# jonaselgammal/GPry

Measured on AMD Instinct MI355X. Metric: gp_refit_plus_nora_acq_cycle_throughput, higher is better.
Workload: dtype f64

## Files before the change

gpry_amd/csrc/api.hip:

```cpp
#include "sweep.h"
#include "kb_gram.h"
#include <algorithm>

int require_model(gpry_ctx* ctx, bool need_factor) {
    if (ctx->N <= 0) return gpry_fail(ctx, -1, "no training set (call gpry_set_train)");
    if (!ctx->have_theta) return gpry_fail(ctx, -1, "no hyperparameters (call gpry_set_theta)");
    if (need_factor && !ctx->factor_valid) return gpry_fail(ctx, -1, "model not factorised (call gpry_factorize)");
    if (need_factor && ctx->tf.has_x_affine)
        for (int k = 0; k < ctx->d; k++)
            if (!(ctx->tf.x_span[k] != 0.0) || !isfinite(ctx->tf.x_span[k]) || !isfinite(ctx->tf.x_lo[k]))
                return gpry_fail(ctx, -1, "affine map of X: span %g, offset %g in dimension %d of %d (gpry_set_affine of another model?)",
                                 ctx->tf.x_span[k], ctx->tf.x_lo[k], k, ctx->d);
    return 0;
}


static int copy_out_matrix(gpry_ctx* ctx, const double* dsrc, int64_t ld, int64_t rows, int64_t cols, double* hdst) {
    HIP_TRY(ctx, hipMemcpy2DAsync(hdst, sizeof(double) * cols, dsrc, sizeof(double) * ld,
                                  sizeof(double) * cols, rows, hipMemcpyDeviceToHost, ctx->stream));
    HIP_TRY(ctx, hipStreamSynchronize(ctx->stream));
    return 0;
}

bool panel_timed_out(int marker) { return (marker & 0xFF00) == 0x5A00; }
// ... 42 lines not shown
                StageScope s(ctx, "trtri");
                if (piped) { GPRY_TRY(trtri_pipeline_finish(ctx)); guard.armed = false; }
                else GPRY_TRY(trtri_lower(ctx, A, V, T, ctx->Np));
            }
        }
    }
    ctx->info_cleared = false;
    if (!info_host) return 0;
    int info[4] = {0, 0, 0, 0};
    HIP_TRY(ctx, hipMemcpyAsync(info, ctx->dinfo, 4 * sizeof(int), hipMemcpyDeviceToHost, ctx->stream));
    HIP_TRY(ctx, hipStreamSynchronize(ctx->stream));
    if (panel_timed_out(info[3])) return panel_timeout_error(ctx, info[3]);
    *info_host = info[0] != 0 ? info[0] : info[1];
    return 0;
}

constexpr int RES_INFO = LML_RES_INFO;
static_assert(RES_INFO + 3 <= GPRY_BRES_STRIDE, "result row too short");
int lml_chain(gpry_ctx* ctx, int want_grad, double* dres) {
    GPRY_TRY(build_factor(ctx, ctx->dW, ctx->dW2, ctx->dW3, nullptr));
    double* dz = ctx->dvec;
    double* da = ctx->dvec + ctx->Np;
    double* dout = ctx->dvec + 2 * ctx->Np;
    {
        StageScope s(ctx, "solve_alpha");
        GPRY_TRY(solve_alpha(ctx, ctx->dW2, ctx->dy, dz, da, ctx->Np));
        GPRY_TRY(logdet_and_quad(ctx, ctx->dW, dz, ctx->Np, dout, want_grad ? nullptr : dres, RES_INFO));
    }
    if (!want_grad) return 0;
    {
        StageScope s(ctx, "lauum");
        GPRY_TRY(lauum_lower(ctx, ctx->dW2, ctx->dW3, ctx->Np));
    }
    StageScope s(ctx, "lml_traces");
    return launch_lml_traces(ctx, ctx->dW3, da, dout + 2, dout, dres, RES_INFO);
}

struct BatchLayout {
    int64_t w, w2, w3, xs, vec, part, split, par, info;
    int64_t part_cap, split_cap, stride;
};
static int batch_layout(gpry_ctx* ctx, const BatchChain& bc, BatchLayout* L) {
    const int64_t Np = ctx->Np, nn = Np * Np;
    int slices = 0;
    GPRY_TRY(factor_chain_slices(ctx, Np, &slices));
    const int DPsel = ctx->d <= 4 ? 4 : ctx->d <= 8 ? 8 : ctx->d <= 16 ? 16 : ctx->d <= 24 ? 24 : 32;
    const int64_t nb = Np / 64, ntile = nb * (nb + 1) / 2;
    const int64_t p1 = ((Np + 255) / 256) * Np, p2 = ntile * (DPsel + 2);
    int64_t o = 0;
    auto take = [&](int64_t n) { const int64_t at = o; o += round_up(n, 32); return at; };
    L->w = take(nn); L->w2 = take(nn); L->w3 = take(nn);
    L->xs = take(Np * ctx->dpad);
    L->vec = take(8 * Np + 4096);
    L->part_cap = p1 > p2 ? p1 : p2;
    if (L->part_cap < bc.part_min) L->part_cap = bc.part_min;
// ... 981 lines not shown
```

gpry_amd/csrc/common.h:

```cpp
#pragma once
#include <hip/hip_runtime.h>
#include <stdint.h>
#include <stdio.h>
#include <string.h>
#include <math.h>
#include <string>
#include <vector>
#include <map>

#include "../../include/gpry_hip.h"

#define GPRY_THETA_MAX (2 + GPRY_MAX_DIM)
#define GPRY_BPAR_ROW (2 + GPRY_MAX_DIM)
#define GPRY_BPAR_WHITE (1 + GPRY_MAX_DIM)
#define GPRY_TILE 128
#define GPRY_NB 64

typedef double v4d __attribute__((ext_vector_type(4)));

struct StageTimer {
    double total_ms = 0.0;
    int64_t count = 0;
    std::vector<std::pair<hipEvent_t, hipEvent_t>> pending;
};

struct FinishParams {
    double C, y_mean, y_std, clip_hi, zeta, baseline, sigma_n;
    int want_std, want_acq;
};

struct gpry_ctx {
    int device = 0;
    hipStream_t stream = nullptr;
// ... 106 lines not shown
    gpry_cand* dcand = nullptr; int64_t cand_cap = 0;
    unsigned long long* dsel = nullptr;
    enum { DSEL_NAN = 0,
           DSEL_STATE = 0,
           DSEL_EMIT = 4,
           DSEL_SURV = 6,
           DSEL_GIDX = 7,
           DSEL_LIVE = 8,
           DSEL_FALL = 9,
           DSEL_WORDS = 64 };

    int64_t kb_n = 0, kb_cap = 0;
    int64_t kb_ld = 0;
    double* dU = nullptr;
    double* dXkb = nullptr;
    double* dkbout = nullptr;

    double* dbord = nullptr;
    int64_t bord_cap = 0;
    int64_t n_border = 0;

    void* trtri_plan = nullptr;
    void* trtri_pipe = nullptr;
    int64_t opt_gemm_streamk = 5632;
    int64_t opt_topk_host = 16384;
    int opt_factor_pipeline = 1;
    int opt_factor_pipeline_min = 1280;
    void* chol_plan = nullptr;

    void* srv = nullptr;
    int opt_predict_serve = 1;
    int64_t opt_serve_idle_us = 2000;
    int opt_mcmc_mapped = 0;
    int64_t opt_chol_stacked = 2048;
    int opt_chol_stacked_dense = 0;
    int opt_sweep_overlap = 0;
    int opt_sweep_upload = 1;
    const double* up_X = nullptr;
    const double* up_y = nullptr;
    int up_gates = 0;
    int opt_kb_rank = 1;
    int opt_predict_gates = 0;
    int opt_sweep_prune = 0;
    int opt_sweep_mean_bound = 1;
    int opt_sweep_screen = 1;
    int sw_pruned = 0;
// ... 68 lines not shown
    return gpry_fail(ctx, -1, "%s: a model with a white term (WhiteKernel, GPRY_KERNEL_WHITE) is not supported by this entry point", who);
}

#define HIP_TRY(ctx, expr)                                                          \
    do {                                                                            \
        hipError_t _e = (expr);                                                     \
        if (_e != hipSuccess)                                                       \
            return gpry_fail(ctx, -2, "%s failed: %s (%s:%d)", #expr,               \
                             hipGetErrorString(_e), __FILE__, __LINE__);            \
    } while (0)

#define GPRY_TRY(expr)                 \
    do {                               \
        int _r = (expr);               \
        if (_r != 0) return _r;        \
    } while (0)

struct StageScope {
    gpry_ctx* ctx; const char* name; hipEvent_t e0 = nullptr, e1 = nullptr; hipStream_t st = nullptr; bool marked = false;
    StageScope(gpry_ctx* c, const char* n, hipStream_t stream = nullptr);
    ~StageScope();
};
void timers_collect(gpry_ctx* ctx);

template <typename T>
int dev_alloc(gpry_ctx* ctx, T** p, int64_t count);
int dev_free(gpry_ctx* ctx, void* p);

static inline int64_t round_up(int64_t a, int64_t b) { return (a + b - 1) / b * b; }
template <typename T>
int dev_grow(gpry_ctx* ctx, T** p, int64_t* cap, int64_t need) {
    if (need <= *cap) return 0;
    HIP_TRY(ctx, hipStreamSynchronize(ctx->stream));
    if (*p) GPRY_TRY(dev_free(ctx, *p));
    *p = nullptr; *cap = 0;
    GPRY_TRY(dev_alloc(ctx, p, need));
    *cap = need;
    return 0;
}

template <typename T>
__device__ __forceinline__ T* bset(T* p, int tb, int64_t bstride) {
    return (T*)((char*)p + (int64_t)tb * bstride * 8);
}
#define GPRY_BRES_STRIDE 40

enum GemmKMode {
    KM_FULL = 0,
    KM_A_LOWER = 1,
    KM_B_LOWER = 2,
    KM_AT_LOWER_B_LOWER = 3,
    KM_B_UPPER = 4,
    KM_AT_LOWER = 5
};
enum GemmEpi { EPI_STORE = 0, EPI_STORE_NEG = 1, EPI_SUB = 2, EPI_SUMSQ = 3 };
enum GemmTileMap { TM_ROWMAJOR = 0, TM_SWEEP = 1, TM_BALANCED = 2 };
#define TM_SWEEP_SMALL (1 << 12)

struct GemmBatchItem { int64_t a_off, b_off, c_off; int M, N, K, pad; };

struct GemmArgs {
    const double* A; const double* B; double* C;
    int64_t lda, ldb, ldc;
    int M, N, K;
    int kmode;
    int lower_only;
    int tile_map;
    const GemmBatchItem* batch;
    int n_batch;
    const int* info;
    hipStream_t stream;
    int nsplit;
    double* split_buf; int64_t split_stride;
    int dma_ok;
    int skip_reduce;
    int small64;
    int bn, bz_div;
    int64_t bstride;
};
__device__ __forceinline__ void gemm_block_z(const GemmArgs& g, int z, int* tb, int* item) {
    if (g.bn > 1) { *tb = z / g.bz_div; *item = z - *tb * g.bz_div; }
    else { *tb = 0; *item = z; }
}
__device__ __forceinline__ bool gemm_block_order(const GemmArgs& g, int* bx, int* tb, int* item) {
    if (g.bn > 1) {
        const int lin = (int)blockIdx.x + (int)gridDim.x * (int)blockIdx.z;
        const int rest = lin / g.bn;
        *tb = lin - rest * g.bn;
        *bx = rest / g.bz_div;
        *item = rest - *bx * g.bz_div;
        return true;
    }
    *bx = (int)blockIdx.x; *tb = 0; *item = (int)blockIdx.z;
    return true;
}
static inline unsigned gemm_grid_z(const GemmArgs& g) { return (unsigned)(g.bz_div * g.bn); }
static inline void gemm_fill_batch(const gpry_ctx* ctx, GemmArgs* g) {
    g->bn = ctx->bn; g->bstride = ctx->bstride; g->bz_div = g->batch ? g->n_batch : 1;
}
struct GemmPart { int bz, ti, tj, lo, hi, slice; };
struct GemmRedTile { int bz, ti, tj, nslice; };
struct GemmPartsPlan {
    GemmPart* d_parts = nullptr; int* d_first = nullptr; GemmRedTile* d_red = nullptr;
    int nwg = 0, nred = 0, max_slices = 0;
};
struct GemmShape { int M, N, K; };
int gemm_parts_segment(int kmode, int lower_only, const std::vector<GemmShape>& shapes, int slots);
int gemm_parts_plan_build(gpry_ctx* ctx, int kmode, int lower_only, const std::vector<GemmShape>& items, int seg_pairs,
                          GemmPartsPlan* out);
void gemm_parts_plan_free(GemmPartsPlan* pl);
int gemm_dma_parts_launch(gpry_ctx* ctx, const GemmArgs& g, bool a_trans, bool b_trans, int epi, const GemmPartsPlan& pl,
                          int64_t slice_stride);
int gemm_f64_launch(gpry_ctx* ctx, const GemmArgs& g, bool a_trans, bool b_trans, int epi);
int gemm64_launch(gpry_ctx* ctx, const GemmArgs& g, bool a_trans, bool b_trans, int epi);
int gemm_split_scratch(gpry_ctx* ctx, int nsplit, int64_t slice, double** buf);
int launch_trtri_diag(gpry_ctx* ctx, const double* L, double* V, int64_t Np, hipStream_t st, bool zero_right = false);
int ensure_pred_xs(gpry_ctx* ctx);
int launch_point_full(gpry_ctx* ctx, const double* x, int want_kinv, double* kstar, double* G, double* u, double* part,
                      double* mean_part, double* ss_part, double* out);
int launch_trtri_diag128(gpry_ctx* ctx, const double* L, double* V, int64_t Np, hipStream_t st, bool clear_right);
int launch_trtri_diag_range(gpry_ctx* ctx, const double* L, double* V, int64_t Np, int blk0, int nblk, hipStream_t st);
bool gemm_dma_usable(const GemmArgs& g, int M, int N, int K);
int gemm_dma_launch_product(gpry_ctx* ctx, const GemmArgs& g, bool a_trans, bool b_trans, int epi, dim3 grid);
int sweep_gemm_dma_sp_launch(gpry_ctx* ctx, const GemmArgs& g);

int upload_params(gpry_ctx* ctx, const double* theta);
int launch_scale_train(gpry_ctx* ctx);
int launch_kernel_train(gpry_ctx* ctx, double* K, int add_noise, double* U = nullptr);
int launch_kernel_rows(gpry_ctx* ctx, int64_t row0, int k, int64_t ldk, double* Bk, double* Cb);
// ... 69 lines not shown
```

gpry_amd/csrc/ctx.hip:

```cpp
#include "common.h"
#include <string>
#include <stdarg.h>
#include <dlfcn.h>

thread_local char g_last_error[1024] = {0};
void trtri_plan_free(gpry_ctx* ctx);
void overlap_plan_free(gpry_ctx* ctx);

int gpry_fail(gpry_ctx* ctx, int code, const char* fmt, ...) {
    va_list ap;
    va_start(ap, fmt);
    vsnprintf(g_last_error, sizeof(g_last_error), fmt, ap);
    va_end(ap);
    if (ctx) { strncpy(ctx->err, g_last_error, sizeof(ctx->err) - 1); }
    return code;
}

template <typename T>
int dev_alloc(gpry_ctx* ctx, T** p, int64_t count) {
    *p = nullptr;
    if (count <= 0) count = 1;
    HIP_TRY(ctx, hipMalloc((void**)p, sizeof(T) * (size_t)count));
    return 0;
}
// ... 229 lines not shown
    HIP_TRY(ctx, hipStreamSynchronize(ctx->stream));
    return 0;
}

namespace {
struct OptionSpec {
    const char* key;
    int64_t lo, hi;
    int64_t (*get)(const gpry_ctx*);
    void (*set)(gpry_ctx*, int64_t);
};
#define OPT_INT(KEY, FIELD, LO, HI, AFTER)                                                         \
    {KEY, LO, HI, [](const gpry_ctx* c) -> int64_t { return (int64_t)c->FIELD; },                  \
     [](gpry_ctx* c, int64_t v) { c->FIELD = (decltype(c->FIELD))v; AFTER; }}
const int64_t BIG = (int64_t)1 << 40;
const OptionSpec OPTIONS[] = {
    OPT_INT("timing", opt_timing, 0, 1, (void)0),
    OPT_INT("chol", opt_chol, 0, 1, c->lml_cache = false),
    OPT_INT("chol_overlap", opt_chol_overlap, 0, 1, c->lml_cache = false),
    OPT_INT("factor_pipeline", opt_factor_pipeline, 0, 1, (void)0),
    OPT_INT("factor_pipeline_min", opt_factor_pipeline_min, 0, BIG, (void)0),
    OPT_INT("gemm_dma", opt_gemm_dma, 0, 1, (void)0),
    OPT_INT("gemm_streamk", opt_gemm_streamk, 0, BIG, trtri_plan_free(c)),
    OPT_INT("gemm_small", opt_gemm_small, 0, BIG, c->lml_cache = false),
    OPT_INT("cross_mfma", opt_cross_mfma, 0, 1, (void)0),
    OPT_INT("cross_hybrid", opt_cross_hybrid, 0, 1, (void)0),
    OPT_INT("sweep_chunk", opt_sweep_chunk, 0, BIG, c->opt_sweep_chunk = round_up(c->opt_sweep_chunk, 1024)),
    OPT_INT("topk_host", opt_topk_host, 0, BIG, (void)0),
    OPT_INT("lml_small", opt_lml_small, 0, 1, c->lml_cache = false),
    OPT_INT("lml_cache", opt_lml_cache, 0, 1, c->lml_cache = false),
    OPT_INT("lml_batch", opt_lml_batch, 0, BIG, (void)0),
    OPT_INT("lml_batch_mb", opt_lml_batch_mb, 1, BIG, (void)0),
    OPT_INT("lml_schedule", opt_lml_schedule, 0, 1, (void)0),
    OPT_INT("lml_streams", opt_lml_streams, 1, 8, (void)0),
    OPT_INT("chol_tp_segments", opt_chol_tp_segments, 0, 1, c->lml_cache = false),
    OPT_INT("panel_debug", opt_panel_debug, 0, 511, c->lml_cache = false),
    OPT_INT("tp_left", opt_tp_left, 0, 1, (void)0),
    OPT_INT("tp_block", opt_tp_block, 128, BIG, c->opt_tp_block = round_up(c->opt_tp_block, 128); overlap_plan_free(c)),
    OPT_INT("tp_tail", opt_tp_tail, 128, BIG, c->opt_tp_tail = round_up(c->opt_tp_tail, 128); overlap_plan_free(c)),
    OPT_INT("predict_small", opt_predict_small, 0, BIG, (void)0),
    OPT_INT("predict_split", opt_predict_split, 0, 1, (void)0),
    OPT_INT("sweep_upload", opt_sweep_upload, 0, 1, (void)0),
    OPT_INT("sweep_overlap", opt_sweep_overlap, 0, 1, (void)0),
    OPT_INT("sweep_prune", opt_sweep_prune, 0, 1, (void)0),
    OPT_INT("sweep_mean_bound", opt_sweep_mean_bound, 0, 1, (void)0),
    OPT_INT("sweep_screen", opt_sweep_screen, 0, 1, (void)0),
// ... 399 lines not shown
```

gpry_amd/csrc/gemm_dma.hip:

```cpp
#include "common.h"
#include <algorithm>

#include "gemm_dma_body.h"

template <bool AT, bool BT, int EPI>
__global__ __launch_bounds__(256, 2) void gemm_dma_kernel(GemmArgs g) {
    constexpr int A_SZ = !AT ? KC_DOUBLES : MC_DOUBLES, B_SZ = BT ? KC_DOUBLES : MC_DOUBLES;
    __shared__ __attribute__((aligned(16))) double smem[2 * (A_SZ + B_SZ)];
    int bx, tb, bz;
    if (!gemm_block_order(g, &bx, &tb, &bz)) return;
    gemm_dma_tile_body<AT, BT, EPI>(g, smem, bx, (int)blockIdx.y, bz, nullptr, tb);
}

bool gemm_dma_usable(const GemmArgs& g, int M, int N, int K) {
    if (M <= 0 || N <= 0 || K < 32) return false;
    if (M % BM || N % BN || K % 32) return false;
    if ((g.lda | g.ldb | g.ldc) & 1) return false;
    return true;
}

template <bool AT, bool BT>
static int gd_launch_epi(gpry_ctx* ctx, const GemmArgs& g, int epi, dim3 grid) {
    hipStream_t st = g.stream ? g.stream : ctx->stream;
    switch (epi) {
// ... 1 lines not shown
        case EPI_STORE_NEG: hipLaunchKernelGGL((gemm_dma_kernel<AT, BT, EPI_STORE_NEG>), grid, dim3(256), 0, st, g); break;
        case EPI_SUB: hipLaunchKernelGGL((gemm_dma_kernel<AT, BT, EPI_SUB>), grid, dim3(256), 0, st, g); break;
        default: return gpry_fail(ctx, -1, "gemm_dma: bad epilogue %d", epi);
    }
    HIP_TRY(ctx, hipGetLastError());
    return 0;
}

int gemm_dma_launch_product(gpry_ctx* ctx, const GemmArgs& g0, bool a_trans, bool b_trans, int epi, dim3 grid) {
    GemmArgs g = g0;
    gemm_fill_batch(ctx, &g);
    grid.z = gemm_grid_z(g);
    if ((g.tile_map & 15) == TM_ROWMAJOR) {
        g.tile_map = TM_BALANCED;
        const int tm = g.M / BM, tn = g.N / BN;
        if (g.lower_only && tm == tn && g.batch == nullptr) grid.x = (unsigned)(tm * (tm + 1) / 2);
    }
    if (!a_trans && !b_trans) return gd_launch_epi<false, false>(ctx, g, epi, grid);
    if (!a_trans && b_trans) return gd_launch_epi<false, true>(ctx, g, epi, grid);
    if (a_trans && !b_trans) return gd_launch_epi<true, false>(ctx, g, epi, grid);
    return gpry_fail(ctx, -1, "gemm_dma: the TT layout is not built");
}

template <bool AT, bool BT, int EPI>
__global__ __launch_bounds__(256, 2) void gemm_dma_parts_kernel(GemmArgs g, const GemmPart* __restrict__ parts,
                                                                const int* __restrict__ first) {
    constexpr int A_SZ = !AT ? KC_DOUBLES : MC_DOUBLES, B_SZ = BT ? KC_DOUBLES : MC_DOUBLES;
    __shared__ __attribute__((aligned(16))) double smem[2 * (A_SZ + B_SZ)];
    const int p1 = first[blockIdx.x + 1];
    for (int p = first[blockIdx.x]; p < p1; p++) {
        const GemmPart pt = parts[p];
        gemm_dma_tile_body<AT, BT, EPI>(g, smem, 0, 0, 0, &pt, (int)blockIdx.z);
        asm volatile("s_waitcnt vmcnt(0) lgkmcnt(0)" ::: "memory");
        __syncthreads();
    }
}

__global__ __launch_bounds__(256) void gemm_parts_reduce_kernel(GemmArgs g, const GemmRedTile* __restrict__ tiles, double sign) {
    const int tb = (int)blockIdx.z;
    if (g.info != nullptr && *bset(g.info, tb, g.bstride) != 0) return;
    const GemmRedTile t = tiles[blockIdx.x];
    const double* split_buf = bset(g.split_buf, tb, g.bstride);
    double* Cb = bset(g.C, tb, g.bstride);
    int64_t coff = 0;
    if (g.batch != nullptr) coff = g.batch[t.bz].c_off;
    const int row0 = t.ti * BM, col0 = t.tj * BN;
    const int rbeg = (int)blockIdx.y * (BM / 8);
    for (int e = threadIdx.x; e < (BM / 8) * (BN / 2); e += 256) {
        const int rr = rbeg + e / (BN / 2), cc = (e % (BN / 2)) * 2;
        const int64_t off = coff + (int64_t)(row0 + rr) * g.ldc + col0 + cc;
        double2 acc = make_double2(0.0, 0.0);
        for (int sidx = 0; sidx < t.nslice; sidx++) {
            const double2 v = *reinterpret_cast<const double2*>(split_buf + (int64_t)sidx * g.split_stride + off);
            acc.x += v.x; acc.y += v.y;
        }
        *reinterpret_cast<double2*>(Cb + off) = make_double2(sign * acc.x, sign * acc.y);
    }
}

namespace {
struct HostTile { int ti, tj, pairs; };
void enumerate_tiles(int kmode, int lower_only, const GemmShape& it, std::vector<HostTile>& out) {
    out.clear();
    const int tm = it.M / BM, tn = it.N / BN;
    for (int ti = 0; ti < tm; ti++)
        for (int tj = 0; tj < tn; tj++) {
            if (lower_only && tj > ti) continue;
            const int row0 = ti * BM, col0 = tj * BN;
            int kbeg = 0, kend = it.K;
            if (kmode == KM_A_LOWER) kend = std::min(it.K, row0 + BM);
            else if (kmode == KM_B_LOWER) kbeg = std::min(it.K, col0);
            else if (kmode == KM_AT_LOWER_B_LOWER) kbeg = std::min(it.K, std::max(row0, col0));
            else if (kmode == KM_B_UPPER) kend = std::min(it.K, col0 + BN);
            else if (kmode == KM_AT_LOWER) kbeg = std::min(it.K, row0);
            out.push_back({ti, tj, (kend - kbeg) / (2 * BK)});
        }
    std::stable_sort(out.begin(), out.end(), [](const HostTile& a, const HostTile& b) { return a.pairs > b.pairs; });
}
}

int gemm_parts_segment(int kmode, int lower_only, const std::vector<GemmShape>& shapes, int slots) {
    int64_t total = 0;
    std::vector<HostTile> tl;
    for (const GemmShape& it : shapes) {
        enumerate_tiles(kmode, lower_only, it, tl);
        for (const HostTile& t : tl) total += t.pairs;
    }
    int64_t seg = (total + slots - 1) / slots;
    if (seg < 4) seg = 4;
    return (int)seg;
}

void gemm_parts_plan_free(GemmPartsPlan* pl) {
    if (pl->d_parts) (void)hipFree(pl->d_parts);
    if (pl->d_first) (void)hipFree(pl->d_first);
    if (pl->d_red) (void)hipFree(pl->d_red);
    *pl = GemmPartsPlan();
}

int gemm_parts_plan_build(gpry_ctx* ctx, int kmode, int lower_only, const std::vector<GemmShape>& items, int seg_pairs,
                          GemmPartsPlan* out) {
    *out = GemmPartsPlan();
    std::vector<GemmPart> parts;
    std::vector<int> first;
    std::vector<GemmRedTile> red;
    std::vector<HostTile> tl;
    int max_slices = 0;
    for (size_t z = 0; z < items.size(); z++) {
        if (items[z].M % BM || items[z].N % BN || items[z].K % (2 * BK))
            return gpry_fail(ctx, -1, "gemm parts: item %zu is not 128-aligned", z);
        enumerate_tiles(kmode, lower_only, items[z], tl);
        int room = 0;
        for (const HostTile& t : tl) {
            if (t.pairs == 0) {
                if (room == 0) { first.push_back((int)parts.size()); room = seg_pairs; }
                parts.push_back({(int)z, t.ti, t.tj, 0, 0, -1});
                continue;
            }
            int done = 0, nslice = 0;
            const size_t p0 = parts.size();
            while (done < t.pairs) {
                if (room == 0) { first.push_back((int)parts.size()); room = seg_pairs; }
                const int take = std::min(room, t.pairs - done);
                parts.push_back({(int)z, t.ti, t.tj, done, done + take, nslice});
                done += take; room -= take; nslice++;
            }
            if (nslice == 1) parts[p0].slice = -1;
            else { red.push_back({(int)z, t.ti, t.tj, nslice}); if (nslice > max_slices) max_slices = nslice; }
        }
        room = 0;
    }
    first.push_back((int)parts.size());
    out->nwg = (int)first.size() - 1;
    out->nred = (int)red.size();
    out->max_slices = max_slices;
    if (out->nwg == 0) return 0;
    hipError_t e = hipMalloc((void**)&out->d_parts, parts.size() * sizeof(GemmPart));
    if (e == hipSuccess) e = hipMalloc((void**)&out->d_first, first.size() * sizeof(int));
    if (e == hipSuccess && !red.empty()) e = hipMalloc((void**)&out->d_red, red.size() * sizeof(GemmRedTile));
    if (e == hipSuccess) e = hipMemcpy(out->d_parts, parts.data(), parts.size() * sizeof(GemmPart), hipMemcpyHostToDevice);
    if (e == hipSuccess) e = hipMemcpy(out->d_first, first.data(), first.size() * sizeof(int), hipMemcpyHostToDevice);
    if (e == hipSuccess && !red.empty()) e = hipMemcpy(out->d_red, red.data(), red.size() * sizeof(GemmRedTile), hipMemcpyHostToDevice);
    if (e != hipSuccess) {
        gemm_parts_plan_free(out);
        return gpry_fail(ctx, -2, "gemm parts plan: %s", hipGetErrorString(e));
    }
    return 0;
}

template <bool AT, bool BT>
static int gd_parts_launch_epi(gpry_ctx* ctx, const GemmArgs& g, int epi, const GemmPartsPlan& pl, hipStream_t st) {
    const dim3 grid((unsigned)pl.nwg, 1, (unsigned)(g.bn > 1 ? g.bn : 1));
    switch (epi) {
        case EPI_STORE: hipLaunchKernelGGL((gemm_dma_parts_kernel<AT, BT, EPI_STORE>), grid, dim3(256), 0, st, g, pl.d_parts, pl.d_first); break;
        case EPI_STORE_NEG: hipLaunchKernelGGL((gemm_dma_parts_kernel<AT, BT, EPI_STORE_NEG>), grid, dim3(256), 0, st, g, pl.d_parts, pl.d_first); break;
        default: return gpry_fail(ctx, -1, "gemm parts: store epilogues only (got %d)", epi);
    }
    HIP_TRY(ctx, hipGetLastError());
    return 0;
}

int gemm_dma_parts_launch(gpry_ctx* ctx, const GemmArgs& g0, bool a_trans, bool b_trans, int epi, const GemmPartsPlan& pl,
                          int64_t slice_stride) {
    if (pl.nwg == 0) return 0;
    GemmArgs g = g0;
    gemm_fill_batch(ctx, &g);
    g.nsplit = 1; g.split_buf = nullptr; g.split_stride = slice_stride;
    if (pl.max_slices > 0) GPRY_TRY(gemm_split_scratch(ctx, pl.max_slices, slice_stride, &g.split_buf));
    hipStream_t st = g.stream ? g.stream : ctx->stream;
    int rc;
    if (!a_trans && !b_trans) rc = gd_parts_launch_epi<false, false>(ctx, g, epi, pl, st);
    else if (!a_trans && b_trans) rc = gd_parts_launch_epi<false, true>(ctx, g, epi, pl, st);
    else if (a_trans && !b_trans) rc = gd_parts_launch_epi<true, false>(ctx, g, epi, pl, st);
    else return gpry_fail(ctx, -1, "gemm parts: the TT layout is not built");
    if (rc || pl.nred == 0) return rc;
    hipLaunchKernelGGL(gemm_parts_reduce_kernel, dim3((unsigned)pl.nred, 8, (unsigned)(g.bn > 1 ? g.bn : 1)), dim3(256), 0, st, g, pl.d_red,
                       epi == EPI_STORE_NEG ? -1.0 : 1.0);
    HIP_TRY(ctx, hipGetLastError());
    return 0;
}
```

gpry_amd/csrc/gemm_dma_body.h:

```cpp
#pragma once
#include "common.h"

#define BM 128
#define BN 128
#define BK 16
#define SMC 144
#define KC_DOUBLES 2048
#define MC_DOUBLES 2304
#define KC_MI_BYTES (16 * 16 * 8)
#define MC_KSTEP_BYTES (4 * SMC * 8)

typedef const __attribute__((address_space(1))) void* gptr_t;
typedef __attribute__((address_space(3))) void* lptr_t;

__device__ __forceinline__ void gd_dma16(const double* g, double* l) {
    __builtin_amdgcn_global_load_lds((gptr_t)g, (lptr_t)l, 16, 0, 0);
}

struct GdFrag { double a0, a1, a2, a3, b0, b1, b2, b3; };

template <bool AKC, bool BKC, int BUF, int KK>
__device__ __forceinline__ void gd_load_frag(GdFrag& f, unsigned addrA, unsigned addrB) {
    constexpr int a_sz = (AKC ? KC_DOUBLES : MC_DOUBLES) * 8, b_sz = (BKC ? KC_DOUBLES : MC_DOUBLES) * 8;
    constexpr int buf_all = BUF * (a_sz + b_sz);
// ... 18 lines not shown
    asm volatile("s_waitcnt lgkmcnt(%8)"
                 : "+v"(f.a0), "+v"(f.a1), "+v"(f.a2), "+v"(f.a3), "+v"(f.b0), "+v"(f.b1), "+v"(f.b2), "+v"(f.b3)
                 : "n"(NPEND) : "memory");
}
__device__ __forceinline__ void gd_mma_frag(v4d (&acc)[4][4], const GdFrag& f) {
    const double a[4] = {f.a0, f.a1, f.a2, f.a3};
    const double b[4] = {f.b0, f.b1, f.b2, f.b3};
#pragma unroll
    for (int mi = 0; mi < 4; mi++)
#pragma unroll
        for (int ni = 0; ni < 4; ni++)
            acc[mi][ni] = __builtin_amdgcn_mfma_f64_16x16x4f64(a[mi], b[ni], acc[mi][ni], 0, 0, 0);
}
__device__ __forceinline__ void gd_mma_row(v4d (&acc)[4][4], const GdFrag& f, int mi) {
    const double a = mi == 0 ? f.a0 : mi == 1 ? f.a1 : mi == 2 ? f.a2 : f.a3;
    acc[mi][0] = __builtin_amdgcn_mfma_f64_16x16x4f64(a, f.b0, acc[mi][0], 0, 0, 0);
    acc[mi][1] = __builtin_amdgcn_mfma_f64_16x16x4f64(a, f.b1, acc[mi][1], 0, 0, 0);
    acc[mi][2] = __builtin_amdgcn_mfma_f64_16x16x4f64(a, f.b2, acc[mi][2], 0, 0, 0);
    acc[mi][3] = __builtin_amdgcn_mfma_f64_16x16x4f64(a, f.b3, acc[mi][3], 0, 0, 0);
}

template <bool AT, bool BT, int EPI>
__device__ __forceinline__ void gemm_dma_tile_body(const GemmArgs& g, double* smem, const int bx, const int by, const int bz_,
                                                   const GemmPart* part = nullptr, const int tb = 0) {
    const int bz = part ? part->bz : bz_;
    constexpr bool AKC = !AT, BKC = BT;
    constexpr int A_SZ = AKC ? KC_DOUBLES : MC_DOUBLES, B_SZ = BKC ? KC_DOUBLES : MC_DOUBLES;
    constexpr int BUF_SZ = A_SZ + B_SZ;
    if (g.info != nullptr && *bset(g.info, tb, g.bstride) != 0) return;

    double* const C0 = bset(g.C, tb, g.bstride);
    double* const split0 = bset(g.split_buf, tb, g.bstride);
    const double* A = bset(g.A, tb, g.bstride); const double* B = bset(g.B, tb, g.bstride); double* C = C0;
    int M = g.M, N = g.N, K = g.K;
    if (g.batch != nullptr) {
        GemmBatchItem it = g.batch[bz];
        A += it.a_off; B += it.b_off; C += it.c_off;
        M = it.M; N = it.N; K = it.K;
    }
    const int tiles_m = M / BM, tiles_n = N / BN;
    int ti, tj;
    if (part) { ti = part->ti; tj = part->tj; }
    else {
        const int b = bx;
        if ((g.tile_map & 15) == TM_SWEEP) {
            const int a = (g.tile_map >> 4) & 15, c = 6 - a;
            const int nsi = (tiles_m + (1 << a) - 1) >> a, nsj = (tiles_n + (1 << c) - 1) >> c;
// ... 149 lines not shown
        gd_mma_row(acc, f1, 2);                                                              \
        __builtin_amdgcn_sched_barrier(0);                                                   \
        issue_piece(s2, BUF, 5); issue_piece(s2, BUF, 6); issue_piece(s2, BUF, 7);           \
        __builtin_amdgcn_sched_barrier(0);                                                   \
        gd_mma_row(acc, f1, 3);                                                              \
        __builtin_amdgcn_sched_barrier(0);                                                   \
    }
    for (int s = 0; s < nslab; s += 2) {
        GD_SLAB_STEP(0, s)
        GD_SLAB_STEP(1, s + 1)
    }
#undef GD_SLAB_STEP
    asm volatile("s_waitcnt vmcnt(0) lgkmcnt(0)" ::: "memory");
    }

#pragma unroll
    for (int mi = 0; mi < 4; mi++)
#pragma unroll
        for (int ni = 0; ni < 4; ni++)
#pragma unroll
            for (int q = 0; q < 4; q++) {
                double* p = cbase + (int64_t)(mi * 16 + 4 * q) * g.ldc + ni * 16;
                const double v = acc[mi][ni][q];
                if (EPI == EPI_STORE || partial) *p = v;
                else *p = -v;
            }
}
```

gpry_amd/csrc/sweep.hip:

```cpp
#include "sweep.h"
#include "acq_math.h"
#include <algorithm>

__global__ void logexp_kernel(const double* __restrict__ mu, const double* __restrict__ sd, int64_t n, double zeta,
                              double baseline, double sigma_n, double* __restrict__ acq) {
    int64_t i = (int64_t)blockIdx.x * blockDim.x + threadIdx.x;
    if (i < n) acq[i] = logexp_value(mu[i], sd[i], zeta, baseline, sigma_n);
}
int launch_logexp(gpry_ctx* ctx, const double* mu, const double* sd, int64_t n, double zeta, double baseline, double sigma_n, double* acq) {
    hipLaunchKernelGGL(logexp_kernel, dim3((unsigned)((n + 255) / 256)), dim3(256), 0, ctx->stream, mu, sd, n, zeta, baseline, sigma_n, acq);
    HIP_TRY(ctx, hipGetLastError());
    return 0;
}

__device__ __forceinline__ double sum_partials(const double* __restrict__ part, int nt, int64_t ldp, int64_t col) {
    double s = 0.0;
#pragma unroll 8
    for (int t = 0; t < nt; t++) s += part[(int64_t)t * ldp + col];
    return s;
}
__device__ __forceinline__ double finish_y(double mu_, unsigned mk, const FinishParams& fp) {
    double y = mu_ * fp.y_std + fp.y_mean;
    y = fmin(y, fp.clip_hi);
    if (mk) y = -INFINITY;
// ... 304 lines not shown
    if (panel_from_matrix_pipe(form) && !no_panel) GPRY_TRY(launch_cross_prepare(ctx));
    if (stage_a) ctx->prune.form = form;
    const MeanBound mb = mean_bound_setup(ctx, rq, fp, nt);
    unsigned long long* live_cnt = nullptr;
    if (stage_a) { ctx->prune.ybound = mb.on ? 1 : 0; ctx->prune.live_blocks = 0; ctx->prune.blocks = 0; ctx->prune.cert_blocks = 0; }
    if (mb.on) {
        if (!ctx->dsel) GPRY_TRY(dev_alloc(ctx, &ctx->dsel, gpry_ctx::DSEL_WORDS));
        live_cnt = ctx->dsel + gpry_ctx::DSEL_LIVE;
        HIP_TRY(ctx, hipMemsetAsync(live_cnt, 0, 16, ctx->stream));
        if (getenv("GPRY_HIP_DEBUG_PANEL"))
            fprintf(stderr, "gpry: bound pass: u in [%.6g, %.3g] skipped, D %.3g, gamma %.3g\n", mb.ubnd, mb.uhi, mb.D1, mb.g3 / 3.0);
    }
    const double* up_X = ctx->up_X;
    const double* up_y = ctx->up_y;
    const size_t nchunk = (size_t)((M + chunk - 1) / chunk);
    if (up_X || overlap) {
        while (ctx->ev_pool.size() < 3 * nchunk + 1) {
            hipEvent_t ev;
            HIP_TRY(ctx, hipEventCreateWithFlags(&ev, hipEventDisableTiming));
            ctx->ev_pool.push_back(ev);
        }
    }
    const hipStream_t main_stream = ctx->stream, side = ctx->stream2;
    struct StreamSwap {
        gpry_ctx* c; hipStream_t keep;
        StreamSwap(gpry_ctx* ctx, hipStream_t st) : c(ctx), keep(ctx->stream) { c->stream = st; }
        ~StreamSwap() { c->stream = keep; }
    };
    auto upload_chunk = [&](size_t ci, bool gates_on_side) -> int {
        const int64_t m0 = (int64_t)ci * chunk, mc = (M - m0 < chunk) ? M - m0 : chunk;
        HIP_TRY(ctx, hipMemcpyAsync(ctx->dXc + m0 * ctx->d, up_X + m0 * ctx->d, sizeof(double) * mc * ctx->d,
                                    hipMemcpyHostToDevice, side));
        if (up_y) HIP_TRY(ctx, hipMemcpyAsync(ctx->dy_all + m0, up_y + m0, sizeof(double) * mc, hipMemcpyHostToDevice, side));
        if (gates_on_side && ctx->up_gates) {
            StreamSwap sw(ctx, side);
            StageScope s(ctx, "gates");
            GPRY_TRY(launch_gates(ctx, ctx->dXc + m0 * ctx->d, mc, ctx->dmask + m0));
        }
        HIP_TRY(ctx, hipEventRecord(ctx->ev_pool[ci], side));
        return 0;
    };
    auto build_panel = [&](size_t ci, double* Kst, double* mean_part) -> int {
        const int64_t m0 = (int64_t)ci * chunk, mc = (M - m0 < chunk) ? M - m0 : chunk, mcp = round_up(mc, 128);
        StageScope s(ctx, stage_a ? "sweep_mean" : "cross_build");
        if (stage_a) Kst = nullptr;
        if (y_given) mean_part = nullptr;
        if (mb.on) {
            ctx->prune.blocks += (int64_t)((mcp + 255) / 256) * 4 * nt * 16;
            return launch_cross_mean_bound(ctx, ctx->dXc, m0, mcp, mean_part, mean_part + (int64_t)nt_mean * chunk, mb.ubnd, mb.uhi, live_cnt);
        }
        return build_sweep_panel(ctx, form, ctx->dXc, m0, mcp, Kst, mean_part);
// ... 311 lines not shown
```

Before: 68.13 million.

## Fuse stream-K split reduction into parts GEMM via arrival counters; add side-stream alpha solve

The split-K parts GEMM now counts slice arrivals per output tile with an atomic word, and the last workgroup to arrive sums the slice partials itself. This removes the separate reduction kernel launch and its extra pass over the scratch buffer. Partial stores become relaxed atomics, and an acquire fence orders them before the sum. It also adds an option, off by default, to run the alpha solve and log-determinant on a second stream alongside lauum. The cost is serialized tail work inside the GEMM and extra atomic and fence overhead.

Result: no change. 67.87 million (-0.4%).

```diff
diff --git a/gpry_amd/csrc/api.hip b/gpry_amd/csrc/api.hip
--- a/gpry_amd/csrc/api.hip
+++ b/gpry_amd/csrc/api.hip
@@ -88,15 +88,37 @@
     double* dz = ctx->dvec;
     double* da = ctx->dvec + ctx->Np;
     double* dout = ctx->dvec + 2 * ctx->Np;
-    {
+    auto alpha_logdet = [&]() -> int {
         StageScope s(ctx, "solve_alpha");
         GPRY_TRY(solve_alpha(ctx, ctx->dW2, ctx->dy, dz, da, ctx->Np));
-        GPRY_TRY(logdet_and_quad(ctx, ctx->dW, dz, ctx->Np, dout, want_grad ? nullptr : dres, RES_INFO));
-    }
+        return logdet_and_quad(ctx, ctx->dW, dz, ctx->Np, dout, want_grad ? nullptr : dres, RES_INFO);
+    };
+    const bool side = want_grad && ctx->opt_alpha_side && ctx->bn == 1 && !ctx->tp && ctx->stream2 != nullptr;
+    struct SideGuard {
+        gpry_ctx* c; bool armed = false;
+        ~SideGuard() { if (armed) (void)hipStreamSynchronize(c->stream2); }
+    } guard{ctx};
+    if (side) {
+        while (ctx->ev_pool.size() < 2) {
+            hipEvent_t ev;
+            HIP_TRY(ctx, hipEventCreateWithFlags(&ev, hipEventDisableTiming));
+            ctx->ev_pool.push_back(ev);
+        }
+        HIP_TRY(ctx, hipEventRecord(ctx->ev_pool[0], ctx->stream));
+        HIP_TRY(ctx, hipStreamWaitEvent(ctx->stream2, ctx->ev_pool[0], 0));
+        guard.armed = true;
+        StreamSwap sw(ctx, ctx->stream2);
+        GPRY_TRY(alpha_logdet());
+    } else GPRY_TRY(alpha_logdet());
     if (!want_grad) return 0;
     {
         StageScope s(ctx, "lauum");
         GPRY_TRY(lauum_lower(ctx, ctx->dW2, ctx->dW3, ctx->Np));
+    }
+    if (side) {
+        HIP_TRY(ctx, hipEventRecord(ctx->ev_pool[1], ctx->stream2));
+        HIP_TRY(ctx, hipStreamWaitEvent(ctx->stream, ctx->ev_pool[1], 0));
+        guard.armed = false;
     }
     StageScope s(ctx, "lml_traces");
     return launch_lml_traces(ctx, ctx->dW3, da, dout + 2, dout, dres, RES_INFO);
diff --git a/gpry_amd/csrc/common.h b/gpry_amd/csrc/common.h
--- a/gpry_amd/csrc/common.h
+++ b/gpry_amd/csrc/common.h
@@ -9,6 +9,7 @@
 #include <map>
 
 #include "../../include/gpry_hip.h"
+#include "gemm_parts_plan.h"
 
 #define GPRY_THETA_MAX (2 + GPRY_MAX_DIM)
 #define GPRY_BPAR_ROW (2 + GPRY_MAX_DIM)
@@ -161,6 +162,8 @@
 
     void* trtri_plan = nullptr;
     void* trtri_pipe = nullptr;
+    int opt_gemm_fixup = 1;
+    int opt_alpha_side = 0;
     int64_t opt_gemm_streamk = 5632;
     int64_t opt_topk_host = 16384;
     int opt_factor_pipeline = 1;
@@ -275,6 +278,11 @@
     ~StageScope();
 };
 void timers_collect(gpry_ctx* ctx);
+struct StreamSwap {
+    gpry_ctx* c; hipStream_t keep;
+    StreamSwap(gpry_ctx* ctx, hipStream_t st) : c(ctx), keep(ctx->stream) { c->stream = st; }
+    ~StreamSwap() { c->stream = keep; }
+};
 
 template <typename T>
 int dev_alloc(gpry_ctx* ctx, T** p, int64_t count);
@@ -298,14 +306,6 @@
 }
 #define GPRY_BRES_STRIDE 40
 
-enum GemmKMode {
-    KM_FULL = 0,
-    KM_A_LOWER = 1,
-    KM_B_LOWER = 2,
-    KM_AT_LOWER_B_LOWER = 3,
-    KM_B_UPPER = 4,
-    KM_AT_LOWER = 5
-};
 enum GemmEpi { EPI_STORE = 0, EPI_STORE_NEG = 1, EPI_SUB = 2, EPI_SUMSQ = 3 };
 enum GemmTileMap { TM_ROWMAJOR = 0, TM_SWEEP = 1, TM_BALANCED = 2 };
 #define TM_SWEEP_SMALL (1 << 12)
@@ -351,13 +351,11 @@
 static inline void gemm_fill_batch(const gpry_ctx* ctx, GemmArgs* g) {
     g->bn = ctx->bn; g->bstride = ctx->bstride; g->bz_div = g->batch ? g->n_batch : 1;
 }
-struct GemmPart { int bz, ti, tj, lo, hi, slice; };
-struct GemmRedTile { int bz, ti, tj, nslice; };
 struct GemmPartsPlan {
     GemmPart* d_parts = nullptr; int* d_first = nullptr; GemmRedTile* d_red = nullptr;
     int nwg = 0, nred = 0, max_slices = 0;
-};
-struct GemmShape { int M, N, K; };
+    mutable unsigned* d_words = nullptr; mutable int64_t words_cap = 0;
+};
 int gemm_parts_segment(int kmode, int lower_only, const std::vector<GemmShape>& shapes, int slots);
 int gemm_parts_plan_build(gpry_ctx* ctx, int kmode, int lower_only, const std::vector<GemmShape>& items, int seg_pairs,
                           GemmPartsPlan* out);
diff --git a/gpry_amd/csrc/ctx.hip b/gpry_amd/csrc/ctx.hip
--- a/gpry_amd/csrc/ctx.hip
+++ b/gpry_amd/csrc/ctx.hip
@@ -275,6 +275,8 @@
     OPT_INT("factor_pipeline_min", opt_factor_pipeline_min, 0, BIG, (void)0),
     OPT_INT("gemm_dma", opt_gemm_dma, 0, 1, (void)0),
     OPT_INT("gemm_streamk", opt_gemm_streamk, 0, BIG, trtri_plan_free(c)),
+    OPT_INT("gemm_fixup", opt_gemm_fixup, 0, 1, c->lml_cache = false),
+    OPT_INT("alpha_side", opt_alpha_side, 0, 1, c->lml_cache = false),
     OPT_INT("gemm_small", opt_gemm_small, 0, BIG, c->lml_cache = false),
     OPT_INT("cross_mfma", opt_cross_mfma, 0, 1, (void)0),
     OPT_INT("cross_hybrid", opt_cross_hybrid, 0, 1, (void)0),
diff --git a/gpry_amd/csrc/gemm_dma.hip b/gpry_amd/csrc/gemm_dma.hip
--- a/gpry_amd/csrc/gemm_dma.hip
+++ b/gpry_amd/csrc/gemm_dma.hip
@@ -47,17 +47,71 @@
     return gpry_fail(ctx, -1, "gemm_dma: the TT layout is not built");
 }
 
+
+template <int E>
+__device__ __forceinline__ void gemm_parts_sum_rows(const GemmArgs& g, int tb, int bz, int ti, int tj, int nslice, double sign,
+                                                    int rbeg, int nrow) {
+    const double* split_buf = bset(g.split_buf, tb, g.bstride);
+    double* Cb = bset(g.C, tb, g.bstride);
+    int64_t coff = 0;
+    if (g.batch != nullptr) coff = g.batch[bz].c_off;
+    const int row0 = ti * BM, col0 = tj * BN;
+    for (int e0 = threadIdx.x; e0 < nrow * (BN / 2); e0 += 256 * E) {
+        int64_t off[E];
+        double2 acc[E];
+#pragma unroll
+        for (int u = 0; u < E; u++) {
+            const int e = e0 + 256 * u;
+            const int rr = rbeg + e / (BN / 2), cc = (e % (BN / 2)) * 2;
+            off[u] = coff + (int64_t)(row0 + rr) * g.ldc + col0 + cc;
+            acc[u] = make_double2(0.0, 0.0);
+        }
+        for (int sidx = 0; sidx < nslice; sidx++) {
+            const double* sp = split_buf + (int64_t)sidx * g.split_stride;
+            double2 v[E];
+#pragma unroll
+            for (int u = 0; u < E; u++) v[u] = *reinterpret_cast<const double2*>(sp + off[u]);
+#pragma unroll
+            for (int u = 0; u < E; u++) { acc[u].x += v[u].x; acc[u].y += v[u].y; }
+        }
+#pragma unroll
+        for (int u = 0; u < E; u++) *reinterpret_cast<double2*>(Cb + off[u]) = make_double2(sign * acc[u].x, sign * acc[u].y);
+    }
+}
+
 template <bool AT, bool BT, int EPI>
 __global__ __launch_bounds__(256, 2) void gemm_dma_parts_kernel(GemmArgs g, const GemmPart* __restrict__ parts,
-                                                                const int* __restrict__ first) {
+                                                                const int* __restrict__ first, unsigned* words, int nred) {
     constexpr int A_SZ = !AT ? KC_DOUBLES : MC_DOUBLES, B_SZ = BT ? KC_DOUBLES : MC_DOUBLES;
     __shared__ __attribute__((aligned(16))) double smem[2 * (A_SZ + B_SZ)];
+    const int tb = (int)blockIdx.z;
     const int p1 = first[blockIdx.x + 1];
     for (int p = first[blockIdx.x]; p < p1; p++) {
         const GemmPart pt = parts[p];
-        gemm_dma_tile_body<AT, BT, EPI>(g, smem, 0, 0, 0, &pt, (int)blockIdx.z);
+        gemm_dma_tile_body<AT, BT, EPI>(g, smem, 0, 0, 0, &pt, tb, words != nullptr);
         asm volatile("s_waitcnt vmcnt(0) lgkmcnt(0)" ::: "memory");
         __syncthreads();
+        if (words == nullptr || pt.slice < 0) continue;
+        unsigned* const word = words + (int64_t)tb * nred + pt.word;
+        volatile int* const flag = reinterpret_cast<volatile int*>(smem);
+        if (threadIdx.x == 0) {
+            const int last = atomicAdd(word, 1u) == (unsigned)(pt.nslice - 1);
+            if (last) {
+                __builtin_amdgcn_fence(__ATOMIC_ACQUIRE, "agent");
+                asm volatile("s_waitcnt vmcnt(0)" ::: "memory");
+            }
+            flag[0] = last;
+        }
+        __syncthreads();
+        const int last = __builtin_amdgcn_readfirstlane(flag[0]);
+        __syncthreads();
+        if (!last) continue;
+        if (g.info == nullptr || *bset(g.info, tb, g.bstride) == 0) {
+            const double sign = EPI == EPI_STORE_NEG ? -1.0 : 1.0;
+            static_assert(BM * (BN / 2) % (256 * 16) == 0, "a thread adds 16 elements per round");
+            gemm_parts_sum_rows<16>(g, tb, pt.bz, pt.ti, pt.tj, pt.nslice, sign, 0, BM);
+        }
+        if (threadIdx.x == 0) __hip_atomic_store(word, 0u, __ATOMIC_RELAXED, __HIP_MEMORY_SCOPE_AGENT);
     }
 }
 
@@ -65,51 +119,15 @@
     const int tb = (int)blockIdx.z;
     if (g.info != nullptr && *bset(g.info, tb, g.bstride) != 0) return;
     const GemmRedTile t = tiles[blockIdx.x];
-    const double* split_buf = bset(g.split_buf, tb, g.bstride);
-    double* Cb = bset(g.C, tb, g.bstride);
-    int64_t coff = 0;
-    if (g.batch != nullptr) coff = g.batch[t.bz].c_off;
-    const int row0 = t.ti * BM, col0 = t.tj * BN;
-    const int rbeg = (int)blockIdx.y * (BM / 8);
-    for (int e = threadIdx.x; e < (BM / 8) * (BN / 2); e += 256) {
-        const int rr = rbeg + e / (BN / 2), cc = (e % (BN / 2)) * 2;
-        const int64_t off = coff + (int64_t)(row0 + rr) * g.ldc + col0 + cc;
-        double2 acc = make_double2(0.0, 0.0);
-        for (int sidx = 0; sidx < t.nslice; sidx++) {
-            const double2 v = *reinterpret_cast<const double2*>(split_buf + (int64_t)sidx * g.split_stride + off);
-            acc.x += v.x; acc.y += v.y;
-        }
-        *reinterpret_cast<double2*>(Cb + off) = make_double2(sign * acc.x, sign * acc.y);
-    }
-}
-
-namespace {
-struct HostTile { int ti, tj, pairs; };
-void enumerate_tiles(int kmode, int lower_only, const GemmShape& it, std::vector<HostTile>& out) {
-    out.clear();
-    const int tm = it.M / BM, tn = it.N / BN;
-    for (int ti = 0; ti < tm; ti++)
-        for (int tj = 0; tj < tn; tj++) {
-            if (lower_only && tj > ti) continue;
-            const int row0 = ti * BM, col0 = tj * BN;
-            int kbeg = 0, kend = it.K;
-            if (kmode == KM_A_LOWER) kend = std::min(it.K, row0 + BM);
-            else if (kmode == KM_B_LOWER) kbeg = std::min(it.K, col0);
-            else if (kmode == KM_AT_LOWER_B_LOWER) kbeg = std::min(it.K, std::max(row0, col0));
-            else if (kmode == KM_B_UPPER) kend = std::min(it.K, col0 + BN);
-            else if (kmode == KM_AT_LOWER) kbeg = std::min(it.K, row0);
-            out.push_back({ti, tj, (kend - kbeg) / (2 * BK)});
-        }
-    std::stable_sort(out.begin(), out.end(), [](const HostTile& a, const HostTile& b) { return a.pairs > b.pairs; });
-}
+    gemm_parts_sum_rows<1>(g, tb, t.bz, t.ti, t.tj, t.nslice, sign, (int)blockIdx.y * (BM / 8), BM / 8);
 }
 
 int gemm_parts_segment(int kmode, int lower_only, const std::vector<GemmShape>& shapes, int slots) {
     int64_t total = 0;
-    std::vector<HostTile> tl;
+    std::vector<GemmHostTile> tl;
     for (const GemmShape& it : shapes) {
-        enumerate_tiles(kmode, lower_only, it, tl);
-        for (const HostTile& t : tl) total += t.pairs;
+        gemm_parts_enumerate_tiles(kmode, lower_only, it, tl);
+        for (const GemmHostTile& t : tl) total += t.pairs;
     }
     int64_t seg = (total + slots - 1) / slots;
     if (seg < 4) seg = 4;
@@ -120,52 +138,36 @@
     if (pl->d_parts) (void)hipFree(pl->d_parts);
     if (pl->d_first) (void)hipFree(pl->d_first);
     if (pl->d_red) (void)hipFree(pl->d_red);
+    if (pl->d_words) (void)hipFree(pl->d_words);
     *pl = GemmPartsPlan();
 }
 
+static hipError_t parts_words_alloc(int64_t n, unsigned** out) {
+    const std::vector<unsigned> zeros((size_t)n, 0u);
+    hipError_t e = hipMalloc((void**)out, (size_t)n * sizeof(unsigned));
+    if (e == hipSuccess) e = hipMemcpy(*out, zeros.data(), (size_t)n * sizeof(unsigned), hipMemcpyHostToDevice);
+    return e;
+}
+
+static_assert(BM == GEMM_PARTS_TILE && BN == GEMM_PARTS_TILE && 2 * BK == GEMM_PARTS_PAIR, "gemm_parts_plan.h cuts other tiles");
 int gemm_parts_plan_build(gpry_ctx* ctx, int kmode, int lower_only, const std::vector<GemmShape>& items, int seg_pairs,
                           GemmPartsPlan* out) {
     *out = GemmPartsPlan();
-    std::vector<GemmPart> parts;
-    std::vector<int> first;
-    std::vector<GemmRedTile> red;
-    std::vector<HostTile> tl;
-    int max_slices = 0;
-    for (size_t z = 0; z < items.size(); z++) {
-        if (items[z].M % BM || items[z].N % BN || items[z].K % (2 * BK))
-            return gpry_fail(ctx, -1, "gemm parts: item %zu is not 128-aligned", z);
-        enumerate_tiles(kmode, lower_only, items[z], tl);
-        int room = 0;
-        for (const HostTile& t : tl) {
-            if (t.pairs == 0) {
-                if (room == 0) { first.push_back((int)parts.size()); room = seg_pairs; }
-                parts.push_back({(int)z, t.ti, t.tj, 0, 0, -1});
-                continue;
-            }
-            int done = 0, nslice = 0;
-            const size_t p0 = parts.size();
-            while (done < t.pairs) {
-                if (room == 0) { first.push_back((int)parts.size()); room = seg_pairs; }
-                const int take = std::min(room, t.pairs - done);
-                parts.push_back({(int)z, t.ti, t.tj, done, done + take, nslice});
-                done += take; room -= take; nslice++;
-            }
-            if (nslice == 1) parts[p0].slice = -1;
-            else { red.push_back({(int)z, t.ti, t.tj, nslice}); if (nslice > max_slices) max_slices = nslice; }
-        }
-        room = 0;
-    }
-    first.push_back((int)parts.size());
-    out->nwg = (int)first.size() - 1;
-    out->nred = (int)red.size();
-    out->max_slices = max_slices;
+    GemmPartsHost h;
+    const int bad = gemm_parts_plan_host(kmode, lower_only, items, seg_pairs, &h);
+    if (bad > 0) return gpry_fail(ctx, -1, "gemm parts: item %d is not 128-aligned", bad - 1);
+    if (bad < 0) return gpry_fail(ctx, -1, "gemm parts: segment length %d", seg_pairs);
+    out->nwg = (int)h.first.size() - 1;
+    out->nred = (int)h.red.size();
+    out->max_slices = h.max_slices;
     if (out->nwg == 0) return 0;
-    hipError_t e = hipMalloc((void**)&out->d_parts, parts.size() * sizeof(GemmPart));
-    if (e == hipSuccess) e = hipMalloc((void**)&out->d_first, first.size() * sizeof(int));
-    if (e == hipSuccess && !red.empty()) e = hipMalloc((void**)&out->d_red, red.size() * sizeof(GemmRedTile));
-    if (e == hipSuccess) e = hipMemcpy(out->d_parts, parts.data(), parts.size() * sizeof(GemmPart), hipMemcpyHostToDevice);
-    if (e == hipSuccess) e = hipMemcpy(out->d_first, first.data(), first.size() * sizeof(int), hipMemcpyHostToDevice);
-    if (e == hipSuccess && !red.empty()) e = hipMemcpy(out->d_red, red.data(), red.size() * sizeof(GemmRedTile), hipMemcpyHostToDevice);
+    hipError_t e = hipMalloc((void**)&out->d_parts, h.parts.size() * sizeof(GemmPart));
+    if (e == hipSuccess) e = hipMalloc((void**)&out->d_first, h.first.size() * sizeof(int));
+    if (e == hipSuccess && !h.red.empty()) e = hipMalloc((void**)&out->d_red, h.red.size() * sizeof(GemmRedTile));
+    if (e == hipSuccess) e = hipMemcpy(out->d_parts, h.parts.data(), h.parts.size() * sizeof(GemmPart), hipMemcpyHostToDevice);
+    if (e == hipSuccess) e = hipMemcpy(out->d_first, h.first.data(), h.first.size() * sizeof(int), hipMemcpyHostToDevice);
+    if (e == hipSuccess && !h.red.empty()) e = hipMemcpy(out->d_red, h.red.data(), h.red.size() * sizeof(GemmRedTile), hipMemcpyHostToDevice);
+    if (e == hipSuccess && !h.red.empty()) { e = parts_words_alloc(out->nred, &out->d_words); out->words_cap = out->nred; }
     if (e != hipSuccess) {
         gemm_parts_plan_free(out);
         return gpry_fail(ctx, -2, "gemm parts plan: %s", hipGetErrorString(e));
@@ -174,11 +176,11 @@
 }
 
 template <bool AT, bool BT>
-static int gd_parts_launch_epi(gpry_ctx* ctx, const GemmArgs& g, int epi, const GemmPartsPlan& pl, hipStream_t st) {
+static int gd_parts_launch_epi(gpry_ctx* ctx, const GemmArgs& g, int epi, const GemmPartsPlan& pl, hipStream_t st, unsigned* words) {
     const dim3 grid((unsigned)pl.nwg, 1, (unsigned)(g.bn > 1 ? g.bn : 1));
     switch (epi) {
-        case EPI_STORE: hipLaunchKernelGGL((gemm_dma_parts_kernel<AT, BT, EPI_STORE>), grid, dim3(256), 0, st, g, pl.d_parts, pl.d_first); break;
-        case EPI_STORE_NEG: hipLaunchKernelGGL((gemm_dma_parts_kernel<AT, BT, EPI_STORE_NEG>), grid, dim3(256), 0, st, g, pl.d_parts, pl.d_first); break;
+        case EPI_STORE: hipLaunchKernelGGL((gemm_dma_parts_kernel<AT, BT, EPI_STORE>), grid, dim3(256), 0, st, g, pl.d_parts, pl.d_first, words, pl.nred); break;
+        case EPI_STORE_NEG: hipLaunchKernelGGL((gemm_dma_parts_kernel<AT, BT, EPI_STORE_NEG>), grid, dim3(256), 0, st, g, pl.d_parts, pl.d_first, words, pl.nred); break;
         default: return gpry_fail(ctx, -1, "gemm parts: store epilogues only (got %d)", epi);
     }
     HIP_TRY(ctx, hipGetLastError());
@@ -193,12 +195,25 @@
     g.nsplit = 1; g.split_buf = nullptr; g.split_stride = slice_stride;
     if (pl.max_slices > 0) GPRY_TRY(gemm_split_scratch(ctx, pl.max_slices, slice_stride, &g.split_buf));
     hipStream_t st = g.stream ? g.stream : ctx->stream;
+    const bool fixup = pl.nred > 0 && ctx->opt_gemm_fixup;
+    unsigned* words = nullptr;
+    if (fixup) {
+        const int64_t need = (int64_t)pl.nred * (g.bn > 1 ? g.bn : 1);
+        if (need > pl.words_cap) {
+            unsigned* w = nullptr;
+            const hipError_t e = parts_words_alloc(need, &w);
+            if (e != hipSuccess) { if (w) (void)hipFree(w); return gpry_fail(ctx, -2, "gemm parts: arrival words: %s", hipGetErrorString(e)); }
+            if (pl.d_words) (void)hipFree(pl.d_words);
+            pl.d_words = w; pl.words_cap = need;
+        }
+        words = pl.d_words;
+    }
     int rc;
-    if (!a_trans && !b_trans) rc = gd_parts_launch_epi<false, false>(ctx, g, epi, pl, st);
-    else if (!a_trans && b_trans) rc = gd_parts_launch_epi<false, true>(ctx, g, epi, pl, st);
-    else if (a_trans && !b_trans) rc = gd_parts_launch_epi<true, false>(ctx, g, epi, pl, st);
+    if (!a_trans && !b_trans) rc = gd_parts_launch_epi<false, false>(ctx, g, epi, pl, st, words);
+    else if (!a_trans && b_trans) rc = gd_parts_launch_epi<false, true>(ctx, g, epi, pl, st, words);
+    else if (a_trans && !b_trans) rc = gd_parts_launch_epi<true, false>(ctx, g, epi, pl, st, words);
     else return gpry_fail(ctx, -1, "gemm parts: the TT layout is not built");
-    if (rc || pl.nred == 0) return rc;
+    if (rc || pl.nred == 0 || fixup) return rc;
     hipLaunchKernelGGL(gemm_parts_reduce_kernel, dim3((unsigned)pl.nred, 8, (unsigned)(g.bn > 1 ? g.bn : 1)), dim3(256), 0, st, g, pl.d_red,
                        epi == EPI_STORE_NEG ? -1.0 : 1.0);
     HIP_TRY(ctx, hipGetLastError());
diff --git a/gpry_amd/csrc/gemm_dma_body.h b/gpry_amd/csrc/gemm_dma_body.h
--- a/gpry_amd/csrc/gemm_dma_body.h
+++ b/gpry_amd/csrc/gemm_dma_body.h
@@ -64,7 +64,7 @@
 
 template <bool AT, bool BT, int EPI>
 __device__ __forceinline__ void gemm_dma_tile_body(const GemmArgs& g, double* smem, const int bx, const int by, const int bz_,
-                                                   const GemmPart* part = nullptr, const int tb = 0) {
+                                                   const GemmPart* part = nullptr, const int tb = 0, const bool slice_wt = false) {
     const int bz = part ? part->bz : bz_;
     constexpr bool AKC = !AT, BKC = BT;
     constexpr int A_SZ = AKC ? KC_DOUBLES : MC_DOUBLES, B_SZ = BKC ? KC_DOUBLES : MC_DOUBLES;
@@ -260,7 +260,8 @@
             for (int q = 0; q < 4; q++) {
                 double* p = cbase + (int64_t)(mi * 16 + 4 * q) * g.ldc + ni * 16;
                 const double v = acc[mi][ni][q];
-                if (EPI == EPI_STORE || partial) *p = v;
+                if (slice_wt && partial) __hip_atomic_store(p, v, __ATOMIC_RELAXED, __HIP_MEMORY_SCOPE_AGENT);
+                else if (EPI == EPI_STORE || partial) *p = v;
                 else *p = -v;
             }
 }
diff --git a/gpry_amd/csrc/gemm_parts_plan.h b/gpry_amd/csrc/gemm_parts_plan.h
--- /dev/null
+++ b/gpry_amd/csrc/gemm_parts_plan.h
@@ -0,0 +1,82 @@
+#pragma once
+#include <algorithm>
+#include <vector>
+
+enum GemmKMode {
+    KM_FULL = 0,
+    KM_A_LOWER = 1,
+    KM_B_LOWER = 2,
+    KM_AT_LOWER_B_LOWER = 3,
+    KM_B_UPPER = 4,
+    KM_AT_LOWER = 5
+};
+
+struct GemmPart { int bz, ti, tj, lo, hi, slice, word, nslice; };
+struct GemmRedTile { int bz, ti, tj, nslice; };
+struct GemmShape { int M, N, K; };
+
+constexpr int GEMM_PARTS_TILE = 128;
+constexpr int GEMM_PARTS_PAIR = 32;
+
+struct GemmHostTile { int ti, tj, pairs; };
+inline void gemm_parts_enumerate_tiles(int kmode, int lower_only, const GemmShape& it, std::vector<GemmHostTile>& out) {
+    constexpr int T = GEMM_PARTS_TILE;
+    out.clear();
+    const int tm = it.M / T, tn = it.N / T;
+    for (int ti = 0; ti < tm; ti++)
+        for (int tj = 0; tj < tn; tj++) {
+            if (lower_only && tj > ti) continue;
+            const int row0 = ti * T, col0 = tj * T;
+            int kbeg = 0, kend = it.K;
+            if (kmode == KM_A_LOWER) kend = std::min(it.K, row0 + T);
+            else if (kmode == KM_B_LOWER) kbeg = std::min(it.K, col0);
+            else if (kmode == KM_AT_LOWER_B_LOWER) kbeg = std::min(it.K, std::max(row0, col0));
+            else if (kmode == KM_B_UPPER) kend = std::min(it.K, col0 + T);
+            else if (kmode == KM_AT_LOWER) kbeg = std::min(it.K, row0);
+            out.push_back({ti, tj, (kend - kbeg) / GEMM_PARTS_PAIR});
+        }
+    std::stable_sort(out.begin(), out.end(), [](const GemmHostTile& a, const GemmHostTile& b) { return a.pairs > b.pairs; });
+}
+
+struct GemmPartsHost {
+    std::vector<GemmPart> parts;
+    std::vector<int> first;
+    std::vector<GemmRedTile> red;
+    int max_slices = 0;
+};
+inline int gemm_parts_plan_host(int kmode, int lower_only, const std::vector<GemmShape>& items, int seg_pairs, GemmPartsHost* out) {
+    *out = GemmPartsHost();
+    if (seg_pairs < 1) return -1;
+    std::vector<GemmPart>& parts = out->parts;
+    std::vector<int>& first = out->first;
+    std::vector<GemmHostTile> tl;
+    for (size_t z = 0; z < items.size(); z++) {
+        if (items[z].M % GEMM_PARTS_TILE || items[z].N % GEMM_PARTS_TILE || items[z].K % GEMM_PARTS_PAIR) return 1 + (int)z;
+        gemm_parts_enumerate_tiles(kmode, lower_only, items[z], tl);
+        int room = 0;
+        for (const GemmHostTile& t : tl) {
+            if (t.pairs == 0) {
+                if (room == 0) { first.push_back((int)parts.size()); room = seg_pairs; }
+                parts.push_back({(int)z, t.ti, t.tj, 0, 0, -1, -1, 1});
+                continue;
+            }
+            int done = 0, nslice = 0;
+            const size_t p0 = parts.size();
+            while (done < t.pairs) {
+                if (room == 0) { first.push_back((int)parts.size()); room = seg_pairs; }
+                const int take = std::min(room, t.pairs - done);
+                parts.push_back({(int)z, t.ti, t.tj, done, done + take, nslice, -1, 1});
+                done += take; room -= take; nslice++;
+            }
+            if (nslice == 1) parts[p0].slice = -1;
+            else {
+                for (size_t p = p0; p < parts.size(); p++) { parts[p].word = (int)out->red.size(); parts[p].nslice = nslice; }
+                out->red.push_back({(int)z, t.ti, t.tj, nslice});
+                if (nslice > out->max_slices) out->max_slices = nslice;
+            }
+        }
+        room = 0;
+    }
+    first.push_back((int)parts.size());
+    return 0;
+}
diff --git a/gpry_amd/csrc/sweep.hip b/gpry_amd/csrc/sweep.hip
--- a/gpry_amd/csrc/sweep.hip
+++ b/gpry_amd/csrc/sweep.hip
@@ -350,11 +350,6 @@
         }
     }
     const hipStream_t main_stream = ctx->stream, side = ctx->stream2;
-    struct StreamSwap {
-        gpry_ctx* c; hipStream_t keep;
-        StreamSwap(gpry_ctx* ctx, hipStream_t st) : c(ctx), keep(ctx->stream) { c->stream = st; }
-        ~StreamSwap() { c->stream = keep; }
-    };
     auto upload_chunk = [&](size_t ci, bool gates_on_side) -> int {
         const int64_t m0 = (int64_t)ci * chunk, mc = (M - m0 < chunk) ? M - m0 : chunk;
         HIP_TRY(ctx, hipMemcpyAsync(ctx->dXc + m0 * ctx->d, up_X + m0 * ctx->d, sizeof(double) * mc * ctx->d,
```
